# datatypevoid/babble

Hardware: AMD Instinct MI355X
Metric: consensus-ordered events/sec at N=256 peers (1 GPU and 8-GPU batched sims) (higher is better)
Workload: dtype int32

## Files before the change

### babble_amd/_lib.py

```python
from __future__ import annotations

import ctypes as C
import os

import numpy as np

HERE = os.path.dirname(os.path.abspath(__file__))
LIB_PATH = os.path.join(HERE, os.environ.get("HGX_LIB", "libhgx.so"))

_L = None


class HgxError(RuntimeError):

    def __init__(self, code: int, msg: str):
        super().__init__(msg)
        self.code = code
        self.msg = msg


class hgx_error(C.Structure):
    _fields_ = [("code", C.c_int32), ("msg", C.c_char * 252)]


# ... 134 lines not shown
    _sig(L, "hgx_last_round", i32, [p, i32])
    _sig(L, "hgx_round_event_count", i32, [p, i32, i32])
    _sig(L, "hgx_round_witnesses", i32, [p, i32, i32, p, i32])
    _sig(L, "hgx_known", i32, [p, i32, p])
    _sig(L, "hgx_consensus_events_count", i64, [p, i32])
    _sig(L, "hgx_consensus_events", i32, [p, i32, i64, i64, p])
    _sig(L, "hgx_num_blocks", i64, [p, i32])
    _sig(L, "hgx_block_info", i32, [p, i32, i64, p, p, p, p, p, p])
    _sig(L, "hgx_get_block", i32, [p, i32, i32, p, E])
    _sig(L, "hgx_consensus_received", i32, [p, i32, i64, i64, p, p, p])
    _sig(L, "hgx_last_from", i32, [p, i32, p, p, E])
    _sig(L, "hgx_participant_events", i32, [p, i32, i64, p, i64, p, E])
    _sig(L, "hgx_participant_event", i32, [p, i32, i64, p, E])
    _sig(L, "hgx_get_root", i32, [p, i32, p, p, p, p, E])
    _sig(L, "hgx_get_event", i32, [p, i64, p, p, p, p, p, p, p, E])
    _sig(L, "hgx_wire_info", i32, [p, i64, i64, p, p, p])
    _sig(L, "hgx_read_wire_info", i32, [p, i32, i64, i32, i64, p, p, E])
    _sig(L, "hgx_diff_wire", i32, [p, i32, p, i64, p, i64, C.POINTER(C.c_int64), C.POINTER(C.c_int32), E])
    _sig(L, "hgx_keep_bodies", i32, [p, i64, i64, E])
    _sig(L, "hgx_bodies_state", i32, [p, C.POINTER(C.c_int64), C.POINTER(C.c_int64), C.POINTER(C.c_int64)])
    _sig(L, "hgx_get_event_bodies", i32, [p, p, i64, p, p, p, i64, p, i64, C.POINTER(C.c_int64),
                                          C.POINTER(C.c_int64), E])
    _sig(L, "hgx_block_transactions", i32, [p, i32, i64, p, i64, p, i64, C.POINTER(C.c_int64),
                                            C.POINTER(C.c_int64), E])
    _sig(L, "hgx_get_block_hash", i32, [p, i32, i64, p, E])
    _sig(L, "hgx_block_hash_batch", i32, [i32, p, p, p, p, p, i64, p, E])
    _sig(L, "hgx_diff_wire_bodies", i32, [p, i32, p, i64, p, C.POINTER(hgx_wire_body_out), i64, C.POINTER(C.c_int64),
                                          C.POINTER(C.c_int64), C.POINTER(C.c_int64), C.POINTER(C.c_int32), E])
    _sig(L, "hgx_get_rounds", i32, [p, i64, i64, p, p, p])
    _sig(L, "hgx_get_received", i32, [p, i64, i64, p, p])
    _sig(L, "hgx_get_coords", i32, [p, i64, p, p])
    for nm in ("hgx_ancestor", "hgx_self_ancestor", "hgx_see", "hgx_strongly_see", "hgx_round", "hgx_witness"):
        _sig(L, nm, i32, [p, i64, i64] if nm not in ("hgx_round", "hgx_witness") else [p, i64])
    _sig(L, "hgx_oldest_self_ancestor_to_see", i64, [p, i64, i64])
    _sig(L, "hgx_block_hash", i32, [i64, i32, p, p, i32, p])
    _sig(L, "hgx_sha256_batch", i32, [i32, p, p, i64, p, p])
    _sig(L, "hgx_sha256_batch_device", i32, [p, p, i64, p, p])
    _sig(L, "hgx_p256_verify_batch", i32, [i32, p, i32, p, p, p, p, i64, p, p])
    _sig(L, "hgx_p256_verify_bench", i32, [i32, p, i32, p, p, p, p, i64, i32, i32, p, C.POINTER(C.c_double)])
    _sig(L, "hgx_sha256_bench", i32, [i32, i64, i32, i32, C.c_uint64, i32, i32, C.POINTER(C.c_double),
                                      C.POINTER(C.c_int64), C.POINTER(C.c_int64), i64, p])
    _sig(L, "hgx_phase_times", i32, [p, p, i32])
    _sig(L, "hgx_kernel_stats", i32, [p, i32, C.c_char_p, i32, C.POINTER(C.c_double), C.POINTER(C.c_int64),
                                      C.POINTER(C.c_double)])
    _sig(L, "hgx_reset_stats", i32, [p])
    _sig(L, "hgx_set_kernel_timing", i32, [p, i32])
    _sig(L, "hgx_set_coord_storage", i32, [p, i32])
    _sig(L, "hgx_set_fame_tally", i32, [p, i32])
    _sig(L, "hgx_set_round_kernel", i32, [p, i32])
    _sig(L, "hgx_set_sort_kernel", i32, [p, i32])
    _sig(L, "hgx_set_round_shards", i32, [p, i32])
    _sig(L, "hgx_set_shard_remote", i32, [p, i32])
    _sig(L, "hgx_exchange_floor_bench", i32, [i32, i32, i32, i32, C.POINTER(C.c_double)])
    _sig(L, "hgx_set_cts_kernel", i32, [p, i32])
    _sig(L, "hgx_set_root_others", i32, [p, p, i64, p])
    _sig(L, "hgx_set_la_kernel", i32, [p, i32])
    _sig(L, "hgx_set_ingest_pipeline", i32, [p, i32, i64])
    _sig(L, "hgx_set_incremental", i32, [p, i32])
    _sig(L, "hgx_find_order_begin", i32, [p, p])
    _sig(L, "hgx_find_order_end", i32, [p, p])
    _sig(L, "hgx_set_shard", i32, [p, i32, i32])
    _sig(L, "hgx_reset", i32, [p, p, p, p, p])
    _sig(L, "hgx_insert_wire_events", i32, [p, p, i64, p, p])
    _sig(L, "hgx_insert_wire_bodies", i32, [p, C.POINTER(hgx_wire_bodies), i64, p, p, p, C.POINTER(C.c_int64), E])
    _sig(L, "hgx_set_commit_callback", i32, [p, C.c_void_p, p])
    _sig(L, "hgx_get_frame", i32, [p, p, i64, p, p, p, p, p, p, p, i64, p, p])
    _sig(L, "hgx_prune_to_frame", i32, [p, p, i64, C.POINTER(C.c_int64), E])
    _sig(L, "hgx_get_root_ids", i32, [p, i32, p, C.POINTER(C.c_int32), p, C.POINTER(C.c_int32), E])
    _sig(L, "hgx_get_root_others", i32, [p, p, p, i64, C.POINTER(C.c_int64), E])
    _sig(L, "hgx_set_root_ids", i32, [p, p, p, p, p, p, p, i64, E])
    _sig(L, "hgx_shard_values", i64, [p, i32])
    _sig(L, "hgx_shard_export", i32, [p, p, i32])
    _sig(L, "hgx_shard_import", i32, [p, i32, p, i32])
    _sig(L, "hgx_reserve_rounds", i32, [p, i32])
    _sig(L, "hgx_device_alloc", i32, [i32, i64, C.POINTER(C.c_void_p)])
    _sig(L, "hgx_device_free", i32, [i32, p])
    _sig(L, "hgx_device_copy", i32, [i32, p, p, i64, i32])
    _L = L
    return L


def check(rc: int, err: hgx_error):
    if rc != 0:
        raise HgxError(int(err.code or rc), err.msg.decode(errors="replace"))
```

### babble_amd/csrc/hgx_device.h

```cpp
#pragma once

#include <hip/hip_runtime.h>

#include <cstdint>

namespace hgx {

__device__ __forceinline__ int lane_id() { return (int)(threadIdx.x & 63); }

__device__ __forceinline__ uint32_t block_excl_scan256(uint32_t v, uint32_t* sh, uint32_t* total) {
    const int lane = lane_id(), wave = threadIdx.x >> 6;
    uint32_t x = v;
    for (int o = 1; o < 64; o <<= 1) {
        const uint32_t y = __shfl_up(x, o);
        if (lane >= o) x += y;
    }
    if (lane == 63) sh[wave] = x;
    __syncthreads();
    uint32_t wbase = 0;
    for (int w = 0; w < wave; w++) wbase += sh[w];
    *total = sh[0] + sh[1] + sh[2] + sh[3];
    __syncthreads();
    return wbase + x - v;
}

template <int HD>
__device__ __forceinline__ uint32_t swar_ge_count(const uint32_t (&v)[HD], const uint32_t (&nf)[HD]) {
    uint32_t c = 0;
    if constexpr (HD % 2 == 0) {
#pragma unroll
        for (int i = 0; i < HD / 2; i++) {
            const uint64_t s = ((((uint64_t)v[2 * i + 1]) << 32) | v[2 * i]) + ((((uint64_t)nf[2 * i + 1]) << 32) | nf[2 * i]);
            c = __builtin_popcount((uint32_t)s & 0x80808080u) + c;
            asm volatile("" : "+v"(c));
            c = __builtin_popcount((uint32_t)(s >> 32) & 0x80808080u) + c;
            asm volatile("" : "+v"(c));
        }
    } else {
#pragma unroll
        for (int d = 0; d < HD; d++) c += __builtin_popcount((v[d] + nf[d]) & 0x80808080u);
    }
    return c;
}
__device__ __forceinline__ uint32_t swar_nf(uint32_t fd7) { return 0x80808080u - fd7; }

__device__ __forceinline__ uint64_t group_mask(int gs, int grp) {
    return (gs >= 64) ? ~0ull : (((1ull << gs) - 1ull) << (gs * grp));
}

template <typename CT>
struct Coord;
template <>
struct Coord<int32_t> {
    static constexpr int32_t kLaNone = -1;
    __device__ __forceinline__ static int32_t la(int32_t v) { return v; }
    __device__ __forceinline__ static int32_t enc_la(int32_t v) { return v; }
    __device__ __forceinline__ static int32_t fd(int32_t v) { return v; }
    __device__ __forceinline__ static int32_t enc_fd(int32_t v) { return v; }
};
template <>
struct Coord<uint16_t> {
    static constexpr int32_t kLaNone = 0;
    __device__ __forceinline__ static int32_t la(uint32_t v) { return (int32_t)v - 1; }
    __device__ __forceinline__ static uint16_t enc_la(int32_t v) { return (uint16_t)(v + 1); }
    __device__ __forceinline__ static int32_t fd(uint32_t v) { return v == 0xFFFFu ? 2147483647 : (int32_t)v; }
    __device__ __forceinline__ static uint16_t enc_fd(int32_t v) { return v >= 0xFFFF ? (uint16_t)0xFFFF : (uint16_t)v; }
};

__device__ __forceinline__ void wave_lds_fence() {
    __builtin_amdgcn_fence(__ATOMIC_SEQ_CST, "wavefront");
    __builtin_amdgcn_wave_barrier();
}

__device__ __forceinline__ uint64_t wave_min_u64(uint64_t x) {
    for (int o = 32; o >= 1; o >>= 1) {
        const uint64_t y = __shfl_xor(x, o);
        x = y < x ? y : x;
    }
    return x;
}

__device__ __forceinline__ uint64_t wave_max_u64(uint64_t x) {
    for (int o = 32; o >= 1; o >>= 1) {
        const uint64_t y = __shfl_xor(x, o);
        x = y > x ? y : x;
    }
    return x;
}

template <int CPL>
__device__ uint64_t wave_select_kth(const uint64_t (&v)[CPL], const bool (&ok)[CPL], int K,
                                    uint32_t* __restrict__ hist) {
    const int lane = lane_id();
    uint64_t lo = ~0ull, hi = 0;
#pragma unroll
    for (int q = 0; q < CPL; q++)
        if (ok[q]) { lo = v[q] < lo ? v[q] : lo; hi = v[q] > hi ? v[q] : hi; }
    lo = wave_min_u64(lo);
    hi = wave_max_u64(hi);
    bool act[CPL];
#pragma unroll
    for (int q = 0; q < CPL; q++) act[q] = ok[q];
    uint64_t base = lo;
    uint64_t range = hi - lo;
    int k = K;
    while (range != 0) {
        int bits = 64 - __clzll((long long)range);
        const int shift = bits > 8 ? bits - 8 : 0;
#pragma unroll
        for (int t = 0; t < 4; t++) hist[lane * 4 + t] = 0;
        wave_lds_fence();
#pragma unroll
        for (int q = 0; q < CPL; q++)
            if (act[q]) atomicAdd(&hist[(uint32_t)((v[q] - base) >> shift)], 1u);
        wave_lds_fence();
        uint32_t h[4], s = 0;
#pragma unroll
        for (int t = 0; t < 4; t++) { h[t] = hist[lane * 4 + t]; s += h[t]; }
        uint32_t incl = s;
        for (int o = 1; o < 64; o <<= 1) {
            const uint32_t y = __shfl_up(incl, o);
            if (lane >= o) incl += y;
        }
        const uint32_t excl = incl - s;
        int bucket = -1;
        uint32_t below = 0;
// ... 323 lines not shown
```

### babble_amd/csrc/hgx_kernels.hip

```cpp
#include <hip/hip_runtime.h>

#include <algorithm>
#include <cstdint>
#include <cstdlib>
#include <cstring>
#include <map>
#include <mutex>
#include <tuple>

#include "hgx_device.h"
#include "hgx_kernels.h"

namespace hgx {


constexpr int kLayoutB = 4096;
constexpr int kLayoutH = 1024;

__global__ void __launch_bounds__(256) k_ck_pack(int64_t E0, int64_t E, const int32_t* __restrict__ g_creator,
                                                 const int32_t* __restrict__ g_index, const int32_t* __restrict__ c_base,
                                                 int64_t* __restrict__ g_ck, const int32_t* __restrict__ gate) {
    if (gate && *gate) return;
    const int64_t gid = E0 + (int64_t)blockIdx.x * blockDim.x + threadIdx.x;
    if (gid >= E) return;
    const int c = g_creator[gid];
    g_ck[gid] = ((int64_t)c << 32) | (uint32_t)(g_index[gid] - c_base[c]);
}

__device__ __forceinline__ void layout_one(int64_t gid, int p, const int32_t* __restrict__ g_creator,
                                           const int64_t* __restrict__ g_ck, const int32_t* __restrict__ g_op,
                                           const int64_t* __restrict__ g_ts, const int32_t* __restrict__ g_rr,
                                           const int64_t* __restrict__ g_cts, const int32_t* __restrict__ c_off,
                                           const int32_t* __restrict__ c_base, int32_t* __restrict__ p_gid,
                                           int32_t* __restrict__ p_chain, int32_t* __restrict__ p_op,
                                           int32_t* __restrict__ p_opu, int32_t* __restrict__ p_opk,
                                           int64_t* __restrict__ p_ts, int32_t* __restrict__ p_rr,
                                           int64_t* __restrict__ p_cts, int C, int n, int seg) {
    const int c = g_creator[gid];
    const int op = g_op[gid];
    int opp = -1, opu = -1, opk = -1;
    if (op >= 0) {
        const int64_t ck = g_ck[op];
        const int oc = (int)(ck >> 32);
        const int ok = (int)(uint32_t)ck;
        opp = c_off[oc] + ok;
        opu = (ok / seg) * C + oc;
        opk = ((oc % n) << kOpkBits) | (ok & ((1 << kOpkBits) - 1));
    }
    p_opk[p] = opk;
    p_gid[p] = (int32_t)gid;
    p_chain[p] = c;
    p_op[p] = opp;
    p_opu[p] = opu;
    p_ts[p] = g_ts[gid];
    p_rr[p] = g_rr[gid];
    p_cts[p] = g_cts[gid];
}

__global__ void __launch_bounds__(256) k_layout_direct(int64_t E0, int64_t E, const int32_t* __restrict__ g_creator,
                                                       const int32_t* __restrict__ g_index, const int64_t* __restrict__ g_ck,
                                                       const int32_t* __restrict__ g_op,
                                                       const int64_t* __restrict__ g_ts, const int32_t* __restrict__ g_rr,
// ... 1366 lines not shown
                                                          uint32_t* __restrict__ segcur, uint64_t* __restrict__ kout,
                                                          uint32_t* __restrict__ vout) {
    const int i = blockIdx.x * blockDim.x + threadIdx.x;
    const bool v = i < m;
    int seg = -1, p = 0;
    uint64_t key = 0;
    if (v) {
        p = list[i];
        seg = (p_chain[p] / n) * R + p_rr[p];
        key = ((uint64_t)seg << cts_bits) | (uint64_t)(p_cts[p] - cmin);
    }
    bool head;
    int hl, len;
    wave_seg_runs(v, seg, head, hl, len);
    uint32_t base = 0;
    if (head) base = atomicAdd(&segcur[seg], (uint32_t)len);
    base = (uint32_t)__shfl((int)base, hl);
    if (v) {
        const uint32_t slot = segoff[seg] + base + (uint32_t)(lane_id() - hl);
        kout[slot] = key;
        vout[slot] = (uint32_t)p;
    }
}

__global__ void __launch_bounds__(256) k_seg_max(int nseg, const uint32_t* __restrict__ segc,
                                                 unsigned long long* __restrict__ out) {
    uint32_t mx = 0;
    for (int s = blockIdx.x * blockDim.x + threadIdx.x; s < nseg; s += gridDim.x * blockDim.x) mx = max(mx, segc[s]);
    for (int o = 32; o >= 1; o >>= 1) mx = max(mx, (uint32_t)__shfl_xor(mx, o));
    if (lane_id() == 0 && mx) atomicMax(out, (unsigned long long)mx);
}

__device__ __forceinline__ int cmp_s(const uint8_t* a, const uint8_t* b) {
    for (int k = 0; k < 32; k++)
        if (a[k] != b[k]) return a[k] < b[k] ? -1 : 1;
    return 0;
}

struct SortFinish {
    const int32_t* p_rr;
    const int64_t* p_cts;
    const int32_t* g_ntx;
    const uint8_t* g_loaded;
    const uint8_t* g_txnil;
    int32_t* order_gid;
    int32_t* g_rr;
    int64_t* g_cts;
    int32_t* blk_cnt;
    int64_t* blk_ntx;
    int32_t* blk_loaded;
    uint8_t* blk_nil;
};

template <int GS, int TB>
__global__ void __launch_bounds__(TB) k_seg_sort(int nseg, int seg0, int seg1, int32_t m, const uint32_t* __restrict__ segoff,
                                                  const uint64_t* __restrict__ kin, const uint32_t* __restrict__ vin,
                                                  const int32_t* __restrict__ p_gid, const uint8_t* __restrict__ g_S,
                                                  uint32_t* __restrict__ vout, int cap, SortFinish F) {
    extern __shared__ __attribute__((aligned(16))) uint64_t smem[];
    __shared__ int64_t red_ntx[TB / 64];
    __shared__ int32_t red_ld[TB / 64];
    constexpr int NG = TB / GS;
    const int grp = (int)threadIdx.x / GS, t = (int)threadIdx.x % GS;
    uint64_t* sk = smem + (size_t)grp * cap;
    uint32_t* sv = (uint32_t*)(smem + (size_t)NG * cap) + (size_t)grp * cap;
    uint16_t* rs = (uint16_t*)((uint32_t*)(smem + (size_t)NG * cap) + (size_t)NG * cap) + (size_t)grp * 2 * cap;
    auto sync = [&]() {
        if constexpr (GS == 64) wave_lds_fence(); else __syncthreads();
    };
    const int sgi = seg0 + (int)blockIdx.x * NG + grp;
    int o = 0, len = 0;
    if (sgi < seg1) {
        o = (int)segoff[sgi];
        len = (sgi + 1 < nseg ? (int)segoff[sgi + 1] : m) - o;
    }
    int64_t ntx = 0;
    int ld = 0;
    auto emit = [&](int i, uint32_t p) {
        vout[o + i] = p;
        const int gid = p_gid[p];
        F.order_gid[o + i] = gid;
        F.g_rr[gid] = F.p_rr[p];
        F.g_cts[gid] = F.p_cts[p];
        ntx += F.g_ntx[gid];
        ld += F.g_loaded[gid] ? 1 : 0;
        if (i == 0) F.blk_nil[sgi] = F.g_txnil[gid];
    };
    auto block_totals = [&]() {
        for (int w = 32; w >= 1; w >>= 1) {
            ntx += __shfl_xor(ntx, w);
            ld += __shfl_xor(ld, w);
        }
        if constexpr (GS > 64) {
            if (lane_id() == 0) { red_ntx[threadIdx.x >> 6] = ntx; red_ld[threadIdx.x >> 6] = ld; }
            __syncthreads();
            if (threadIdx.x == 0)
                for (int w = 1; w < TB / 64; w++) { ntx += red_ntx[w]; ld += red_ld[w]; }
        }
        if (t == 0 && len > 0) {
            F.blk_cnt[sgi] = len;
            F.blk_ntx[sgi] = ntx;
            F.blk_loaded[sgi] = ld;
        }
    };
    if (len <= 1) {
        if (len == 1 && t == 0) emit(0, vin[o]);
        block_totals();
        return;
    }
    int P = 2;
    while (P < len) P <<= 1;
    for (int i = t; i < P; i += GS) {
        sk[i] = i < len ? kin[o + i] : ~0ull;
        sv[i] = i < len ? vin[o + i] : 0u;
    }
    sync();
    for (int k = 2; k <= P; k <<= 1) {
        for (int j = k >> 1; j > 0; j >>= 1) {
            for (int q = t; q < (P >> 1); q += GS) {
                const int lo = 2 * j * (q / j) + (q & (j - 1)), hi = lo + j;
                const bool asc = (lo & k) == 0;
                const uint64_t a = sk[lo], b = sk[hi];
                if ((a > b) == asc) {
                    sk[lo] = b;
                    sk[hi] = a;
                    const uint32_t x = sv[lo];
                    sv[lo] = sv[hi];
                    sv[hi] = x;
                }
            }
            sync();
        }
    }
    bool tie_any = false;
    for (int i = t; i < len; i += GS) {
        const bool head = i == 0 || sk[i - 1] != sk[i];
        rs[i] = (uint16_t)(head ? i : 0);
        tie_any |= !head;
    }
    if constexpr (GS == 64) tie_any = __any(tie_any); else tie_any = __syncthreads_or(tie_any);
    if (!tie_any) {
        for (int i = t; i < len; i += GS) emit(i, sv[i]);
        block_totals();
        return;
    }
    sync();
    int cur = 0;
    for (int d = 1; d < len; d <<= 1) {
        const uint16_t* src = rs + cur * cap;
        uint16_t* dst = rs + (cur ^ 1) * cap;
        for (int i = t; i < len; i += GS) dst[i] = i >= d ? max(src[i], src[i - d]) : src[i];
        sync();
        cur ^= 1;
    }
    const uint16_t* st = rs + cur * cap;
    for (int i = t; i < len; i += GS) {
        const int s0 = st[i];
        const bool member = s0 != i || (i + 1 < len && st[i + 1] == i);
        if (member) {
            sk[i] = __builtin_bswap64(*(const uint64_t*)(g_S + (size_t)p_gid[sv[i]] * 32));
        }
    }
    sync();
    for (int i = t; i < len; i += GS) {
        const int s0 = st[i];
        const bool member = s0 != i || (i + 1 < len && st[i + 1] == i);
        if (!member) {
            emit(i, sv[i]);
            continue;
        }
        const uint64_t my = sk[i];
        const uint32_t vi = sv[i];
        const uint8_t* si = g_S + (size_t)p_gid[vi] * 32;
        int rank = 0;
        for (int jx = s0; jx < len && st[jx] == s0; jx++) {
            const uint64_t pj = sk[jx];
            const int c = pj != my ? (pj < my ? -1 : 1) : (jx == i ? 0 : cmp_s(g_S + (size_t)p_gid[sv[jx]] * 32, si));
            rank += c < 0 || (c == 0 && jx < i);
        }
        emit(s0 + rank, vi);
    }
    block_totals();
}

__global__ void __launch_bounds__(256) k_minmax_cts(int32_t m, const int32_t* __restrict__ list,
                                                    const int64_t* __restrict__ p_cts,
// ... 631 lines not shown
    const int nb = (m + kSortTile - 1) / kSortTile;
    hipLaunchKernelGGL(k_radix_hist, dim3(nb), dim3(kSortThreads), 0, s, kin, m, shift, a.hist, nb);
    scan_u32(s, a, a.hist, (int64_t)256 * nb);
    hipLaunchKernelGGL(k_radix_scatter, dim3(nb), dim3(kSortThreads), 0, s, kin, vin, m, shift, a.hist, nb, kout,
                       vout);
}

void launch_sort(hipStream_t s, const DevArrays& a, int32_t m, int64_t cmin, int cts_bits, int R, int n,
                 int seg_bits, uint32_t** final_vals, uint64_t** final_keys) {
    uint64_t *ka = a.key_a, *kb = a.key_b;
    uint32_t *va = a.val_a, *vb = a.val_b;
    if (cts_bits + seg_bits <= 64) {
        hipLaunchKernelGGL(k_keys_comb, dim3(nblk(m, 256)), dim3(256), 0, s, m, a.recv_list, a.p_cts, a.p_chain,
                           a.p_rr, cmin, cts_bits, R, n, ka, va);
        for (int sh = 0; sh < cts_bits + seg_bits; sh += 8) {
            radix_pass(s, a, m, sh, ka, va, kb, vb);
            uint64_t* tk = ka; ka = kb; kb = tk;
            uint32_t* tv = va; va = vb; vb = tv;
        }
        hipLaunchKernelGGL(k_tie_prefix, dim3(nblk(m, 256)), dim3(256), 0, s, m, va, ka, a.p_gid, a.g_S, kb);
        hipLaunchKernelGGL(k_tiefix_rank, dim3(nblk(m, 256)), dim3(256), 0, s, m, va, vb, ka, kb, a.p_gid, a.g_S);
        va = vb;
        *final_vals = va;
        *final_keys = ka;
        return;
    }
    hipLaunchKernelGGL(k_keys_cts, dim3(nblk(m, 256)), dim3(256), 0, s, m, a.recv_list, a.p_cts, cmin, ka, va);
    for (int sh = 0; sh < cts_bits; sh += 8) {
        radix_pass(s, a, m, sh, ka, va, kb, vb);
        uint64_t* tk = ka; ka = kb; kb = tk;
        uint32_t* tv = va; va = vb; vb = tv;
    }
    hipLaunchKernelGGL(k_keys_seg, dim3(nblk(m, 256)), dim3(256), 0, s, m, va, a.p_chain, a.p_rr, R, n, ka);
    for (int sh = 0; sh < seg_bits; sh += 8) {
        radix_pass(s, a, m, sh, ka, va, kb, vb);
        uint64_t* tk = ka; ka = kb; kb = tk;
        uint32_t* tv = va; va = vb; vb = tv;
    }
    hipLaunchKernelGGL(k_tiefix, dim3(nblk(m, 256)), dim3(256), 0, s, m, va, ka, a.p_cts, a.p_gid, a.g_S);
    *final_vals = va;
    *final_keys = ka;
}

int seg_sort_cap() { return kSegSortCap; }

void launch_seg_count(hipStream_t s, const DevArrays& a, int32_t m, int R, int n, int nseg, uint32_t* segc,
                      unsigned long long* max_out) {
    hipLaunchKernelGGL(k_seg_count_mm, dim3(std::min(2048u, nblk(m, 256))), dim3(256), 0, s, m, a.recv_list, a.p_cts,
                       a.p_chain, a.p_rr, R, n, segc, (unsigned long long*)a.minmax);
    hipLaunchKernelGGL(k_seg_max, dim3(std::max(1, std::min(256, (nseg + 255) / 256))), dim3(256), 0, s, nseg, segc,
                       max_out);
}

hipError_t launch_sort_seg(hipStream_t s, const DevArrays& a, int32_t m, int64_t cmin, int cts_bits, int R, int n,
                           int nseg, uint32_t* segoff, uint32_t* segcur, int max_seg, uint32_t** final_vals,
                           uint64_t** final_keys, const std::vector<int>* cuts,
                           const std::function<hipError_t(int)>& after_part) {
    uint64_t* kb = a.key_b;
    uint32_t *va = a.val_a, *vb = a.val_b;
    int cap = 2;
    while (cap < max_seg) cap <<= 1;
    if (cap > 512) {
        const hipError_t e = ensure_lds_limit((const void*)k_seg_sort<1024, 1024>, (size_t)cap * 16);
        if (e != hipSuccess) return e;
    }
    scan_u32(s, a, segoff, nseg);
    (void)hipMemsetAsync(segcur, 0, (size_t)nseg * 4, s);
    hipLaunchKernelGGL(k_seg_keys_scatter, dim3(nblk(m, 256)), dim3(256), 0, s, m, a.recv_list, a.p_cts, a.p_chain,
                       a.p_rr, cmin, cts_bits, R, n, segoff, segcur, kb, vb);
    const SortFinish F{a.p_rr, a.p_cts, a.g_ntx, a.g_loaded, a.g_txnil, a.order_gid, a.g_rr, a.g_cts,
                       a.blk_cnt, a.blk_ntx, a.blk_loaded, a.blk_nil};
    const int np = cuts ? (int)cuts->size() - 1 : 1;
    for (int k = 0; k < np; k++) {
        const int s0 = cuts ? (*cuts)[k] : 0, s1 = cuts ? (*cuts)[k + 1] : nseg;
        if (s1 > s0) {
            if (cap <= 512) {
                const size_t lds = (size_t)4 * cap * 16;
                hipLaunchKernelGGL((k_seg_sort<64, 256>), dim3((s1 - s0 + 3) / 4), dim3(256), lds, s, nseg, s0, s1, m,
                                   segoff, kb, vb, a.p_gid, a.g_S, va, cap, F);
            } else {
                const size_t lds = (size_t)cap * 16;
                hipLaunchKernelGGL((k_seg_sort<1024, 1024>), dim3(s1 - s0), dim3(1024), lds, s, nseg, s0, s1, m, segoff,
                                   kb, vb, a.p_gid, a.g_S, va, cap, F);
            }
        }
        if (after_part) {
            const hipError_t e = after_part(k);
            if (e != hipSuccess) return e;
        }
    }
    *final_vals = va;
    *final_keys = kb;
    return hipGetLastError();
}

void launch_root_floor(hipStream_t s, const DevArrays& a, const int32_t* root_round, int32_t* gfl, int32_t* gB,
                       int gmax, int C, int n, int max_len) {
    const int64_t work = (int64_t)C * max_len;
    if (work <= 0 || gmax < 0) return;
    if (a.compact)
        hipLaunchKernelGGL(k_root_floor<uint16_t>, dim3(nblk(work, 256)), dim3(256), 0, s, a.c_off, a.c_len, a.c_base,
                           root_round, (const uint16_t*)a.LA, gfl, C, n, max_len);
    else
        hipLaunchKernelGGL(k_root_floor<int32_t>, dim3(nblk(work, 256)), dim3(256), 0, s, a.c_off, a.c_len, a.c_base,
                           root_round, (const int32_t*)a.LA, gfl, C, n, max_len);
    hipLaunchKernelGGL(k_root_bound_init, dim3(nblk((int64_t)(gmax + 1) * C, 256)), dim3(256), 0, s, gB, a.c_len, C,
                       gmax);
    hipLaunchKernelGGL(k_root_bound, dim3(nblk(work, 256)), dim3(256), 0, s, a.c_off, a.c_len, gfl, gB, C, gmax,
                       max_len);
}

__global__ void k_round_first_gid(int r0, int R, int C, const int32_t* __restrict__ Bm, const uint8_t* __restrict__ wstat,
                                  const int32_t* __restrict__ c_off, const int32_t* __restrict__ p_gid,
                                  int32_t* __restrict__ first) {
    const int64_t t = (int64_t)blockIdx.x * blockDim.x + threadIdx.x;
    if (t >= (int64_t)(R - r0) * C) return;
    const int r = r0 + (int)(t / C), c = (int)(t % C);
    if (wstat[(size_t)r * C + c] != 2) return;
    atomicMin(&first[r - r0], p_gid[c_off[c] + Bm[(size_t)r * C + c]]);
}

void launch_round_first_gid(hipStream_t s, const DevArrays& a, int r0, int R, int C, int32_t* first) {
    if (R <= r0) return;
    hipLaunchKernelGGL(k_round_first_gid, dim3(nblk((int64_t)(R - r0) * C, 256)), dim3(256), 0, s, r0, R, C, a.Bm,
                       a.wstat, a.c_off, a.p_gid, first);
}

bool sort_small_ok(int32_t m) { return m <= kSortSmallMax; }

void launch_sort_small(hipStream_t s, const DevArrays& a, int32_t m, int n, uint32_t** final_vals) {
    const unsigned t = (unsigned)((m + kRankTile - 1) / kRankTile), tj = (unsigned)((m + kRankJT - 1) / kRankJT);
    hipLaunchKernelGGL(k_sort_rank, dim3(t, tj), dim3(kRankTile), 0, s, m, a.recv_list, a.p_cts, a.p_chain, a.p_rr,
                       a.p_gid, a.g_S, n, a.val_b);
    hipLaunchKernelGGL(k_sort_place, dim3(nblk(m, 256)), dim3(256), 0, s, m, a.recv_list, a.val_b, a.val_a);
    *final_vals = a.val_a;
}

void launch_finish_order(hipStream_t s, const DevArrays& a, int32_t m, const uint32_t* vals, int R, int n) {
    hipLaunchKernelGGL(k_finish_order, dim3(nblk(m, 256)), dim3(256), 0, s, m, vals, a.p_gid, a.p_chain, a.p_rr,
                       a.p_cts, a.g_ntx, a.g_loaded, a.g_txnil, R, n, a.order_gid, a.g_rr, a.g_cts, a.blk_cnt,
                       a.blk_ntx, a.blk_loaded, a.blk_nil);
}

void launch_gather_i32(hipStream_t s, int64_t E, const int32_t* src, const int32_t* g_pos, int32_t* dst) {
    if (E <= 0) return;
    hipLaunchKernelGGL(k_gather_i32, dim3(nblk(E, 256)), dim3(256), 0, s, E, src, g_pos, dst);
}
// ... 3 lines not shown
```

### babble_amd/hashgraph.py

```python
from __future__ import annotations

import ctypes as C
import os
from typing import List, Optional, Sequence

import numpy as np

from . import _lib
from ._lib import HgxError, hgx_error, hgx_events, ptr

UNKNOWN_PARENT = -2


def compact_columns(t) -> dict:
    ntx = np.where(np.asarray(t.txnil) != 0, -1, np.asarray(t.ntx)).astype(np.int32)
    return dict(creator=np.ascontiguousarray(t.creator, np.int32), index=np.ascontiguousarray(t.index, np.int32),
                sp=np.ascontiguousarray(t.sp, np.int32), op=np.ascontiguousarray(t.op, np.int32),
                ts=np.ascontiguousarray(t.ts, np.int64),
                coin=np.ascontiguousarray(np.asarray(t.hash)[:, 16] != 0, np.uint8),
                s=np.ascontiguousarray(t.s, np.uint8), ntx=ntx)


class HostBuffer:

# ... 967 lines not shown

def sha256_batch(data: np.ndarray, offsets: np.ndarray, device: int = 0) -> np.ndarray:
    data = np.ascontiguousarray(data, dtype=np.uint8)
    offsets = np.ascontiguousarray(offsets, dtype=np.int64)
    count = max(len(offsets) - 1, 0)
    out = np.zeros((count, 32), dtype=np.uint8)
    err = hgx_error()
    rc = _lib.lib().hgx_sha256_batch(device, ptr(data) if data.size else None, ptr(offsets) if count else None,
                                     count, ptr(out) if count else None, C.byref(err))
    _lib.check(rc, err)
    return out


def event_ids(bodies: Sequence[bytes], device: int = 0) -> List[bytes]:
    lens = np.fromiter((len(b) for b in bodies), dtype=np.int64, count=len(bodies))
    offsets = np.zeros(len(bodies) + 1, dtype=np.int64)
    np.cumsum(lens, out=offsets[1:])
    data = np.frombuffer(b"".join(bodies), dtype=np.uint8)
    return [bytes(r) for r in sha256_batch(data, offsets, device)]


def _splitmix64(x: np.ndarray) -> np.ndarray:
    with np.errstate(over="ignore"):
        z = x + np.uint64(0x9E3779B97F4A7C15)
        z = (z ^ (z >> np.uint64(30))) * np.uint64(0xBF58476D1CE4E5B9)
        z = (z ^ (z >> np.uint64(27))) * np.uint64(0x94D049BB133111EB)
        return z ^ (z >> np.uint64(31))


def sha256_bench_messages(n: int, min_len: int, max_len: int, seed: int) -> List[bytes]:
    i = np.arange(n, dtype=np.uint64)
    lens = min_len + (_splitmix64(~np.uint64(seed) + i) % np.uint64(max_len - min_len + 1)).astype(np.int64)
    total = int(lens.sum())
    words = _splitmix64(np.uint64(seed) + np.arange((total + 7) // 8, dtype=np.uint64))
    blob = words.astype("<u8").tobytes()
    out, o = [], 0
    for ln in lens:
        out.append(blob[o:o + int(ln)])
        o += int(ln)
    return out


def sha256_bench(count: int, min_len: int, max_len: int, seed: int = 5, warmup: int = 1, iters: int = 3,
                 n_sample: int = 64, device: int = 0) -> dict:
    ms, tot, nb = C.c_double(), C.c_int64(), C.c_int64()
    sample = np.zeros((n_sample, 32), dtype=np.uint8)
    rc = _lib.lib().hgx_sha256_bench(device, count, min_len, max_len, seed, warmup, iters, C.byref(ms),
                                     C.byref(tot), C.byref(nb), n_sample, ptr(sample))
    if rc:
        raise HgxError(rc, "hgx_sha256_bench failed")
    return {"ms_per_launch": ms.value, "bytes": tot.value, "blocks": nb.value, "sample": sample}


def _p256_cols(keys65, key_idx, digest, r, s):
    k = np.ascontiguousarray(keys65, np.uint8).reshape(-1, 65)
    cols = [np.ascontiguousarray(key_idx, np.int32)] + [np.ascontiguousarray(x, np.uint8).reshape(-1, 32)
                                                         for x in (digest, r, s)]
    m = cols[0].shape[0]
    assert all(c.shape[0] == m for c in cols[1:])
    return k, cols, m


def p256_verify(keys65, key_idx, digest, r, s, device: int = 0) -> np.ndarray:
    k, cols, m = _p256_cols(keys65, key_idx, digest, r, s)
    out = np.zeros(m, np.uint8)
    err = hgx_error()
    rc = _lib.lib().hgx_p256_verify_batch(device, ptr(k), k.shape[0], *[ptr(c) for c in cols], m, ptr(out),
                                          C.byref(err))
    _lib.check(rc, err)
    return out


def p256_verify_bench(keys65, key_idx, digest, r, s, warmup: int = 1, iters: int = 3, device: int = 0) -> dict:
    k, cols, m = _p256_cols(keys65, key_idx, digest, r, s)
    out = np.zeros(m, np.uint8)
    ms = C.c_double()
    rc = _lib.lib().hgx_p256_verify_bench(device, ptr(k), k.shape[0], *[ptr(c) for c in cols], m, warmup, iters,
                                          ptr(out), C.byref(ms))
    if rc:
        raise HgxError(rc, "hgx_p256_verify_bench failed")
    return {"ms_per_launch": ms.value, "out": out}
```

### include/hgx.h

```cpp
#ifndef HGX_H
#define HGX_H

#include <stdint.h>

#ifdef __cplusplus
extern "C" {
#endif

#define HGX_ABI_VERSION 6

enum {
    HGX_OK = 0,
    HGX_ERR_KEY_NOT_FOUND = 1,
    HGX_ERR_TOO_LATE = 2,
    HGX_ERR_PASSED_INDEX = 3,
    HGX_ERR_SKIPPED_INDEX = 4,
    HGX_ERR_NO_ROOT = 5,
    HGX_ERR_SELF_PARENT = 100,
    HGX_ERR_OTHER_PARENT = 101,
    HGX_ERR_INVALID = 102,
    HGX_ERR_CAPACITY = 103,
    HGX_ERR_SIGNATURE = 104,
    HGX_ERR_DEVICE = 200,
    HGX_ERR_PANIC = 300
// ... 218 lines not shown
} hgx_wire_out;
int32_t hgx_diff_wire(hgx_ctx* ctx, int32_t graph, const int32_t* known, int64_t sync_limit,
                      hgx_wire_out* out, int64_t cap, int64_t* count, int32_t* over_limit, hgx_error* err);

int32_t hgx_keep_bodies(hgx_ctx* ctx, int64_t tx_hint, int64_t bytes_hint, hgx_error* err);
int32_t hgx_bodies_state(hgx_ctx* ctx, int64_t* n_events, int64_t* n_tx, int64_t* n_bytes);
int32_t hgx_get_event_bodies(hgx_ctx* ctx, const int64_t* gids, int64_t count, uint8_t* sig_r, int32_t* ntx,
                             int64_t* tx_off, int64_t tx_cap, uint8_t* tx_bytes, int64_t bytes_cap, int64_t* n_tx,
                             int64_t* n_bytes, hgx_error* err);
int32_t hgx_block_transactions(hgx_ctx* ctx, int32_t graph, int64_t b, int64_t* tx_off, int64_t tx_cap,
                               uint8_t* tx_bytes, int64_t bytes_cap, int64_t* n_tx, int64_t* n_bytes, hgx_error* err);
int32_t hgx_get_block_hash(hgx_ctx* ctx, int32_t graph, int64_t b, uint8_t* out32, hgx_error* err);
int32_t hgx_block_hash_batch(int32_t device, const int64_t* round_received, const int32_t* ntx,
                             const int32_t* tx_nil, const int64_t* tx_off, const uint8_t* tx_bytes, int64_t count,
                             uint8_t* out32, hgx_error* err);
typedef struct {
    uint8_t* sig_r;
    int64_t* tx_off;
    int64_t tx_cap;
    uint8_t* tx_bytes;
    int64_t bytes_cap;
} hgx_wire_body_out;
int32_t hgx_diff_wire_bodies(hgx_ctx* ctx, int32_t graph, const int32_t* known, int64_t sync_limit,
                             hgx_wire_out* out, hgx_wire_body_out* body, int64_t cap, int64_t* count, int64_t* n_tx,
                             int64_t* n_bytes, int32_t* over_limit, hgx_error* err);

int32_t hgx_get_rounds(hgx_ctx* ctx, int64_t first, int64_t count, int32_t* round, int8_t* witness,
                       int8_t* famous);
int32_t hgx_get_received(hgx_ctx* ctx, int64_t first, int64_t count, int32_t* round_received,
                         int64_t* consensus_ts);
int32_t hgx_get_coords(hgx_ctx* ctx, int64_t gid, int32_t* last_ancestors, int32_t* first_descendants);

int32_t hgx_ancestor(hgx_ctx* ctx, int64_t x, int64_t y);
int32_t hgx_self_ancestor(hgx_ctx* ctx, int64_t x, int64_t y);
int32_t hgx_see(hgx_ctx* ctx, int64_t x, int64_t y);
int32_t hgx_strongly_see(hgx_ctx* ctx, int64_t x, int64_t y);
int64_t hgx_oldest_self_ancestor_to_see(hgx_ctx* ctx, int64_t x, int64_t y);
int32_t hgx_round(hgx_ctx* ctx, int64_t x);
int32_t hgx_witness(hgx_ctx* ctx, int64_t x);

int32_t hgx_block_hash(int64_t round_received, int32_t ntx, const uint8_t* const* tx, const int64_t* tx_len,
                       int32_t tx_nil, uint8_t* out32);

int32_t hgx_sha256_batch(int32_t device, const uint8_t* data, const int64_t* offsets, int64_t count,
                         uint8_t* out32, hgx_error* err);
int32_t hgx_sha256_batch_device(const uint8_t* d_data, const int64_t* d_offsets, int64_t count,
                                uint8_t* d_out32, void* stream);
int32_t hgx_sha256_bench(int32_t device, int64_t count, int32_t min_len, int32_t max_len, uint64_t seed,
                         int32_t warmup, int32_t iters, double* ms_per_launch, int64_t* total_bytes,
                         int64_t* n_blocks, int64_t n_sample, uint8_t* sample32);

int32_t hgx_exchange_floor_bench(int32_t device, int32_t chains, int32_t n, int32_t rounds, double* us_per_round);

int32_t hgx_p256_verify_batch(int32_t device, const uint8_t* keys65, int32_t n_keys, const int32_t* key_idx,
                              const uint8_t* digest32, const uint8_t* r32, const uint8_t* s32, int64_t count,
                              uint8_t* out, hgx_error* err);
int32_t hgx_p256_verify_bench(int32_t device, const uint8_t* keys65, int32_t n_keys, const int32_t* key_idx,
                              const uint8_t* digest32, const uint8_t* r32, const uint8_t* s32, int64_t count,
                              int32_t warmup, int32_t iters, uint8_t* out, double* ms_per_launch);

int32_t hgx_phase_times(hgx_ctx* ctx, double* out, int32_t cap);
int32_t hgx_kernel_stats(hgx_ctx* ctx, int32_t k, char* name, int32_t name_cap, double* ms, int64_t* launches,
                         double* bytes);
int32_t hgx_reset_stats(hgx_ctx* ctx);
int32_t hgx_set_kernel_timing(hgx_ctx* ctx, int32_t mask);

int32_t hgx_set_coord_storage(hgx_ctx* ctx, int32_t mode);
int32_t hgx_set_fame_tally(hgx_ctx* ctx, int32_t mode);
int32_t hgx_set_ingest_pipeline(hgx_ctx* ctx, int32_t pieces, int64_t min_events);
int32_t hgx_set_la_kernel(hgx_ctx* ctx, int32_t mode);
int32_t hgx_set_round_kernel(hgx_ctx* ctx, int32_t mode);
int32_t hgx_set_sort_kernel(hgx_ctx* ctx, int32_t mode);
int32_t hgx_set_round_shards(hgx_ctx* ctx, int32_t shards);
int32_t hgx_set_shard_remote(hgx_ctx* ctx, int32_t on);
int32_t hgx_set_cts_kernel(hgx_ctx* ctx, int32_t mode);
int32_t hgx_set_incremental(hgx_ctx* ctx, int32_t on);
int32_t hgx_reserve_rounds(hgx_ctx* ctx, int32_t rounds);

int32_t hgx_device_alloc(int32_t device, int64_t bytes, void** ptr);
int32_t hgx_device_free(int32_t device, void* ptr);
int32_t hgx_device_copy(int32_t device, void* dst, const void* src, int64_t bytes, int32_t to_device);

int32_t hgx_trace_gossip(int32_t n_participants, int32_t n_silent, int64_t n_events, uint64_t seed,
                         double stale_prob, int32_t stale_depth,
                         int32_t* creator, int64_t* index, int64_t* self_parent, int64_t* other_parent,
                         int64_t* timestamp_ns, uint8_t* hash, uint8_t* sig_s, int32_t* ntx, int32_t* tx_nil,
                         int64_t* tx_seq);
int32_t hgx_trace_tx_payload(int32_t creator, int64_t seq, uint8_t* out, int32_t cap);

#ifdef __cplusplus
}
#endif
#endif
```

Measured before the change: 284.8 million.

## Register-resident bitonic segment sort with DPP lane exchanges and packed key-index words

Rewrites the per-segment bitonic sort so each thread holds EPT elements in registers. Intra-thread stages use compare-swaps, intra-wave stages use DPP/swizzle lane exchanges, and only cross-wave stages go through LDS with barriers. When key bits plus log2(cap) fit in 64 bits, the value index is packed into the key's low bits, so only one word moves per compare and values are gathered once at the end. This removes most LDS traffic and barriers from the old shared-memory network, at the cost of a template explosion over EPT and PACK, higher register pressure, and a new host-callable correctness check entry point.

```diff
diff --git a/babble_amd/_lib.py b/babble_amd/_lib.py
--- a/babble_amd/_lib.py
+++ b/babble_amd/_lib.py
@@ -210,6 +210,7 @@
     _sig(L, "hgx_set_round_shards", i32, [p, i32])
     _sig(L, "hgx_set_shard_remote", i32, [p, i32])
     _sig(L, "hgx_exchange_floor_bench", i32, [i32, i32, i32, i32, C.POINTER(C.c_double)])
+    _sig(L, "hgx_seg_sort_check", i32, [i32, i32, p, i32, p, p, p, i32, p, C.POINTER(C.c_int32)])
     _sig(L, "hgx_set_cts_kernel", i32, [p, i32])
     _sig(L, "hgx_set_root_others", i32, [p, p, i64, p])
     _sig(L, "hgx_set_la_kernel", i32, [p, i32])
diff --git a/babble_amd/csrc/hgx_device.h b/babble_amd/csrc/hgx_device.h
--- a/babble_amd/csrc/hgx_device.h
+++ b/babble_amd/csrc/hgx_device.h
@@ -3,6 +3,8 @@
 #include <hip/hip_runtime.h>
 
 #include <cstdint>
+#include <type_traits>
+#include <utility>
 
 namespace hgx {
 
@@ -72,6 +74,29 @@
     __builtin_amdgcn_wave_barrier();
 }
 
+template <int... I, class F>
+__device__ __forceinline__ void static_for_seq(std::integer_sequence<int, I...>, F&& f) {
+    (f(std::integral_constant<int, I>{}), ...);
+}
+template <int N, class F>
+__device__ __forceinline__ void static_for(F&& f) {
+    static_for_seq(std::make_integer_sequence<int, N>{}, f);
+}
+
+template <int D>
+__device__ __forceinline__ uint32_t lane_xor_u32(uint32_t v) {
+    static_assert(D == 1 || D == 2 || D == 4 || D == 8 || D == 16 || D == 32, "lane distance");
+    if constexpr (D == 1) return (uint32_t)__builtin_amdgcn_update_dpp(0, (int)v, 0xB1, 0xF, 0xF, true);
+    else if constexpr (D == 2) return (uint32_t)__builtin_amdgcn_update_dpp(0, (int)v, 0x4E, 0xF, 0xF, true);
+    else if constexpr (D == 8) return (uint32_t)__builtin_amdgcn_update_dpp(0, (int)v, 0x128, 0xF, 0xF, true);
+    else if constexpr (D == 32) return (uint32_t)__shfl_xor((int)v, 32);
+    else return (uint32_t)__builtin_amdgcn_ds_swizzle((int)v, 0x1F | (D << 10));
+}
+template <int D>
+__device__ __forceinline__ uint64_t lane_xor_u64(uint64_t v) {
+    return ((uint64_t)lane_xor_u32<D>((uint32_t)(v >> 32)) << 32) | lane_xor_u32<D>((uint32_t)v);
+}
+
 __device__ __forceinline__ uint64_t wave_min_u64(uint64_t x) {
     for (int o = 32; o >= 1; o >>= 1) {
         const uint64_t y = __shfl_xor(x, o);
diff --git a/babble_amd/csrc/hgx_kernels.hip b/babble_amd/csrc/hgx_kernels.hip
--- a/babble_amd/csrc/hgx_kernels.hip
+++ b/babble_amd/csrc/hgx_kernels.hip
@@ -8,6 +8,7 @@
 #include <mutex>
 #include <tuple>
 
+#include "hgx.h"
 #include "hgx_device.h"
 #include "hgx_kernels.h"
 
@@ -1480,7 +1481,14 @@
     uint8_t* blk_nil;
 };
 
-template <int GS, int TB>
+template <bool PACK>
+__device__ __forceinline__ void seg_cx(uint64_t& a, uint32_t& va, uint64_t b, uint32_t vb, bool keep_min) {
+    const bool take = PACK ? (b < a) == keep_min : (keep_min ? b < a : b > a);
+    a = take ? b : a;
+    if constexpr (!PACK) va = take ? vb : va;
+}
+
+template <int GS, int TB, int EPT, bool PACK>
 __global__ void __launch_bounds__(TB) k_seg_sort(int nseg, int seg0, int seg1, int32_t m, const uint32_t* __restrict__ segoff,
                                                   const uint64_t* __restrict__ kin, const uint32_t* __restrict__ vin,
                                                   const int32_t* __restrict__ p_gid, const uint8_t* __restrict__ g_S,
@@ -1489,6 +1497,8 @@
     __shared__ int64_t red_ntx[TB / 64];
     __shared__ int32_t red_ld[TB / 64];
     constexpr int NG = TB / GS;
+    constexpr int CAP = GS * EPT;
+    constexpr int LOGCAP = __builtin_ctz(CAP);
     const int grp = (int)threadIdx.x / GS, t = (int)threadIdx.x % GS;
     uint64_t* sk = smem + (size_t)grp * cap;
     uint32_t* sv = (uint32_t*)(smem + (size_t)NG * cap) + (size_t)grp * cap;
@@ -1538,28 +1548,103 @@
     }
     int P = 2;
     while (P < len) P <<= 1;
-    for (int i = t; i < P; i += GS) {
-        sk[i] = i < len ? kin[o + i] : ~0ull;
-        sv[i] = i < len ? vin[o + i] : 0u;
-    }
+    const int ib = EPT * t;
+    uint64_t w[EPT];
+    uint32_t v[EPT];
+    static_for<EPT>([&](auto E) {
+        constexpr int e = decltype(E)::value;
+        const int i = ib + e;
+        w[e] = ~0ull;
+        v[e] = 0u;
+        if (i < len) {
+            const uint64_t key = kin[o + i];
+            if constexpr (PACK) {
+                w[e] = (key << LOGCAP) | (uint64_t)i;
+            } else {
+                w[e] = key;
+                v[e] = vin[o + i];
+            }
+        }
+    });
+    [[maybe_unused]] int flip = 0;
+    static_for<LOGCAP>([&](auto LK) {
+        constexpr int k = 2 << decltype(LK)::value;
+        if (k <= P) {
+            static_for<decltype(LK)::value + 1>([&](auto JJ) {
+                constexpr int j = (k >> 1) >> decltype(JJ)::value;
+                if constexpr (j < EPT) {
+                    static_for<EPT>([&](auto E) {
+                        constexpr int e = decltype(E)::value;
+                        if constexpr ((e & j) == 0) {
+                            bool asc;
+                            if constexpr (k < EPT) asc = (e & k) == 0; else asc = (ib & k) == 0;
+                            const bool sw = PACK ? (w[e] > w[e + j]) == asc : (asc ? w[e] > w[e + j] : w[e] < w[e + j]);
+                            const uint64_t a = w[e], b = w[e + j];
+                            w[e] = sw ? b : a;
+                            w[e + j] = sw ? a : b;
+                            if constexpr (!PACK) {
+                                const uint32_t x = v[e], y = v[e + j];
+                                v[e] = sw ? y : x;
+                                v[e + j] = sw ? x : y;
+                            }
+                        }
+                    });
+                } else if constexpr (j < 64 * EPT) {
+                    const bool keep_min = ((ib & j) == 0) == ((ib & k) == 0);
+                    static_for<EPT>([&](auto E) {
+                        constexpr int e = decltype(E)::value;
+                        const uint64_t b = lane_xor_u64<j / EPT>(w[e]);
+                        uint32_t vb = 0u;
+                        if constexpr (!PACK) vb = lane_xor_u32<j / EPT>(v[e]);
+                        seg_cx<PACK>(w[e], v[e], b, vb, keep_min);
+                    });
+                } else {
+                    const bool keep_min = ((ib & j) == 0) == ((ib & k) == 0);
+                    const bool in = ib < P;
+                    if constexpr (PACK) {
+                        uint64_t* xb = smem + (flip ? CAP : 0);
+                        flip ^= 1;
+                        if (in) static_for<EPT>([&](auto E) { xb[ib + decltype(E)::value] = w[decltype(E)::value]; });
+                        __syncthreads();
+                        if (in)
+                            static_for<EPT>([&](auto E) {
+                                constexpr int e = decltype(E)::value;
+                                seg_cx<PACK>(w[e], v[e], xb[(ib ^ j) + e], 0u, keep_min);
+                            });
+                    } else {
+                        if (in)
+                            static_for<EPT>([&](auto E) {
+                                constexpr int e = decltype(E)::value;
+                                sk[ib + e] = w[e];
+                                sv[ib + e] = v[e];
+                            });
+                        __syncthreads();
+                        if (in)
+                            static_for<EPT>([&](auto E) {
+                                constexpr int e = decltype(E)::value;
+                                seg_cx<PACK>(w[e], v[e], sk[(ib ^ j) + e], sv[(ib ^ j) + e], keep_min);
+                            });
+                        __syncthreads();
+                    }
+                }
+            });
+        }
+    });
+    if constexpr (PACK && GS > 64) __syncthreads();
+    static_for<EPT>([&](auto E) {
+        constexpr int e = decltype(E)::value;
+        const int i = ib + e;
+        if (i < len) {
+            if constexpr (PACK) {
+                sk[i] = w[e] >> LOGCAP;
+                sv[i] = vin[o + (int)(w[e] & (uint64_t)(CAP - 1))];
+            } else {
+                sk[i] = w[e];
+                sv[i] = v[e];
+            }
+        }
+    });
     sync();
-    for (int k = 2; k <= P; k <<= 1) {
-        for (int j = k >> 1; j > 0; j >>= 1) {
-            for (int q = t; q < (P >> 1); q += GS) {
-                const int lo = 2 * j * (q / j) + (q & (j - 1)), hi = lo + j;
-                const bool asc = (lo & k) == 0;
-                const uint64_t a = sk[lo], b = sk[hi];
-                if ((a > b) == asc) {
-                    sk[lo] = b;
-                    sk[hi] = a;
-                    const uint32_t x = sv[lo];
-                    sv[lo] = sv[hi];
-                    sv[hi] = x;
-                }
-            }
-            sync();
-        }
-    }
     bool tie_any = false;
     for (int i = t; i < len; i += GS) {
         const bool head = i == 0 || sk[i - 1] != sk[i];
@@ -2297,6 +2382,54 @@
                        max_out);
 }
 
+namespace {
+struct SegSortArgs {
+    int nseg, s0, s1;
+    int32_t m;
+    const uint32_t* segoff;
+    const uint64_t* kin;
+    const uint32_t* vin;
+    const int32_t* p_gid;
+    const uint8_t* g_S;
+    uint32_t* vout;
+    int cap;
+    SortFinish F;
+};
+
+template <int GS, int TB, int EPT, bool PACK>
+hipError_t seg_sort_go(hipStream_t s, const SegSortArgs& g, bool launch) {
+    constexpr int NG = TB / GS;
+    const size_t lds = (size_t)NG * g.cap * 16;
+    if (!launch) return GS > 64 ? ensure_lds_limit((const void*)k_seg_sort<GS, TB, EPT, PACK>, lds) : hipSuccess;
+    hipLaunchKernelGGL((k_seg_sort<GS, TB, EPT, PACK>), dim3((g.s1 - g.s0 + NG - 1) / NG), dim3(TB), lds, s, g.nseg, g.s0,
+                       g.s1, g.m, g.segoff, g.kin, g.vin, g.p_gid, g.g_S, g.vout, g.cap, g.F);
+    return hipSuccess;
+}
+
+template <int GS, int TB, bool PACK>
+hipError_t seg_sort_ept(hipStream_t s, const SegSortArgs& g, bool launch) {
+    switch (std::max(1, g.cap / GS)) {
+        case 1: return seg_sort_go<GS, TB, 1, PACK>(s, g, launch);
+        case 2: return seg_sort_go<GS, TB, 2, PACK>(s, g, launch);
+        case 4: return seg_sort_go<GS, TB, 4, PACK>(s, g, launch);
+        case 8: return seg_sort_go<GS, TB, 8, PACK>(s, g, launch);
+        default: return hipErrorInvalidValue;
+    }
+}
+
+bool seg_sort_packs(int cap, int key_bits) {
+    int lc = 6;
+    while ((1 << lc) < cap) lc++;
+    return key_bits + lc <= 64;
+}
+
+hipError_t seg_sort_run(hipStream_t s, const SegSortArgs& g, bool pack, bool launch) {
+    if (g.cap <= 512)
+        return pack ? seg_sort_ept<64, 256, true>(s, g, launch) : seg_sort_ept<64, 256, false>(s, g, launch);
+    return pack ? seg_sort_ept<1024, 1024, true>(s, g, launch) : seg_sort_ept<1024, 1024, false>(s, g, launch);
+}
+}
+
 hipError_t launch_sort_seg(hipStream_t s, const DevArrays& a, int32_t m, int64_t cmin, int cts_bits, int R, int n,
                            int nseg, uint32_t* segoff, uint32_t* segcur, int max_seg, uint32_t** final_vals,
                            uint64_t** final_keys, const std::vector<int>* cuts,
@@ -2305,30 +2438,24 @@
     uint32_t *va = a.val_a, *vb = a.val_b;
     int cap = 2;
     while (cap < max_seg) cap <<= 1;
-    if (cap > 512) {
-        const hipError_t e = ensure_lds_limit((const void*)k_seg_sort<1024, 1024>, (size_t)cap * 16);
+    if (cap > kSegSortCap) return hipErrorInvalidValue;
+    SegSortArgs g{nseg, 0, nseg, m, segoff, kb, vb, a.p_gid, a.g_S, va, cap,
+                  SortFinish{a.p_rr, a.p_cts, a.g_ntx, a.g_loaded, a.g_txnil, a.order_gid, a.g_rr, a.g_cts,
+                             a.blk_cnt, a.blk_ntx, a.blk_loaded, a.blk_nil}};
+    const bool pack = seg_sort_packs(cap, cts_bits);
+    {
+        const hipError_t e = seg_sort_run(s, g, pack, false);
         if (e != hipSuccess) return e;
     }
     scan_u32(s, a, segoff, nseg);
     (void)hipMemsetAsync(segcur, 0, (size_t)nseg * 4, s);
     hipLaunchKernelGGL(k_seg_keys_scatter, dim3(nblk(m, 256)), dim3(256), 0, s, m, a.recv_list, a.p_cts, a.p_chain,
                        a.p_rr, cmin, cts_bits, R, n, segoff, segcur, kb, vb);
-    const SortFinish F{a.p_rr, a.p_cts, a.g_ntx, a.g_loaded, a.g_txnil, a.order_gid, a.g_rr, a.g_cts,
-                       a.blk_cnt, a.blk_ntx, a.blk_loaded, a.blk_nil};
     const int np = cuts ? (int)cuts->size() - 1 : 1;
     for (int k = 0; k < np; k++) {
-        const int s0 = cuts ? (*cuts)[k] : 0, s1 = cuts ? (*cuts)[k + 1] : nseg;
-        if (s1 > s0) {
-            if (cap <= 512) {
-                const size_t lds = (size_t)4 * cap * 16;
-                hipLaunchKernelGGL((k_seg_sort<64, 256>), dim3((s1 - s0 + 3) / 4), dim3(256), lds, s, nseg, s0, s1, m,
-                                   segoff, kb, vb, a.p_gid, a.g_S, va, cap, F);
-            } else {
-                const size_t lds = (size_t)cap * 16;
-                hipLaunchKernelGGL((k_seg_sort<1024, 1024>), dim3(s1 - s0), dim3(1024), lds, s, nseg, s0, s1, m, segoff,
-                                   kb, vb, a.p_gid, a.g_S, va, cap, F);
-            }
-        }
+        g.s0 = cuts ? (*cuts)[k] : 0;
+        g.s1 = cuts ? (*cuts)[k + 1] : nseg;
+        if (g.s1 > g.s0) (void)seg_sort_run(s, g, pack, true);
         if (after_part) {
             const hipError_t e = after_part(k);
             if (e != hipSuccess) return e;
@@ -2338,6 +2465,83 @@
     *final_keys = kb;
     return hipGetLastError();
 }
+
+hipError_t seg_sort_check_run(hipStream_t s, int nseg, int32_t m, int max_seg, int key_bits, bool force_kv,
+                              const uint32_t* segoff, const uint64_t* kin, const uint32_t* vin, const int32_t* p_gid,
+                              const uint8_t* g_S, uint32_t* vout, const SortFinish& F, bool* packed) {
+    int cap = 2;
+    while (cap < max_seg) cap <<= 1;
+    if (cap > kSegSortCap) return hipErrorInvalidValue;
+    const SegSortArgs g{nseg, 0, nseg, m, segoff, kin, vin, p_gid, g_S, vout, cap, F};
+    *packed = !force_kv && seg_sort_packs(cap, key_bits);
+    hipError_t e = seg_sort_run(s, g, *packed, false);
+    if (e == hipSuccess) e = seg_sort_run(s, g, *packed, true);
+    return e == hipSuccess ? hipGetLastError() : e;
+}
+
+}
+
+extern "C" int32_t hgx_seg_sort_check(int32_t device, int32_t nseg, const uint32_t* segoff, int32_t m,
+                                      const uint64_t* keys, const uint32_t* vals, const uint8_t* S32,
+                                      int32_t force_kv, uint32_t* out_vals, int32_t* packed_out) {
+    if (nseg < 1 || m < 1 || !segoff || !keys || !vals || !S32 || !out_vals) return HGX_ERR_INVALID;
+    int64_t max_seg = 0;
+    uint64_t all = 0;
+    if (segoff[0] != 0) return HGX_ERR_INVALID;
+    for (int sg = 0; sg < nseg; sg++) {
+        const int64_t b = segoff[sg], e = sg + 1 < nseg ? (int64_t)segoff[sg + 1] : (int64_t)m;
+        if (e < b || e > m) return HGX_ERR_INVALID;
+        max_seg = std::max(max_seg, e - b);
+    }
+    for (int32_t i = 0; i < m; i++) {
+        if (vals[i] >= (uint32_t)m) return HGX_ERR_INVALID;
+        all |= keys[i];
+    }
+    if (max_seg > hgx::seg_sort_cap()) return HGX_ERR_INVALID;
+    int key_bits = 0;
+    while (key_bits < 64 && (all >> key_bits) != 0) key_bits++;
+    int prev = 0;
+    (void)hipGetDevice(&prev);
+    if (hipSetDevice(device) != hipSuccess) return HGX_ERR_DEVICE;
+    const size_t M = (size_t)m, NS = (size_t)nseg;
+    const size_t o_keys = 0, o_cts = o_keys + 8 * M, o_gcts = o_cts + 8 * M, o_bntx = o_gcts + 8 * M,
+                 o_S = o_bntx + 8 * NS, o_vin = o_S + 32 * M, o_vout = o_vin + 4 * M, o_gid = o_vout + 4 * M,
+                 o_prr = o_gid + 4 * M, o_ntx = o_prr + 4 * M, o_ogid = o_ntx + 4 * M, o_grr = o_ogid + 4 * M,
+                 o_off = o_grr + 4 * M, o_bcnt = o_off + 4 * NS, o_bld = o_bcnt + 4 * NS, o_ld = o_bld + 4 * NS,
+                 o_nil = o_ld + M, o_bnil = o_nil + M, total = o_bnil + NS;
+    uint8_t* d = nullptr;
+    hipStream_t s = nullptr;
+    bool packed = false;
+    std::vector<int32_t> ident(M);
+    for (int32_t i = 0; i < m; i++) ident[(size_t)i] = i;
+    hipError_t e = hipStreamCreateWithFlags(&s, hipStreamNonBlocking);
+    if (e == hipSuccess) e = hipMalloc((void**)&d, total);
+    if (e == hipSuccess) e = hipMemsetAsync(d, 0, total, s);
+    if (e == hipSuccess) e = hipMemcpyAsync(d + o_keys, keys, 8 * M, hipMemcpyHostToDevice, s);
+    if (e == hipSuccess) e = hipMemcpyAsync(d + o_S, S32, 32 * M, hipMemcpyHostToDevice, s);
+    if (e == hipSuccess) e = hipMemcpyAsync(d + o_vin, vals, 4 * M, hipMemcpyHostToDevice, s);
+    if (e == hipSuccess) e = hipMemcpyAsync(d + o_gid, ident.data(), 4 * M, hipMemcpyHostToDevice, s);
+    if (e == hipSuccess) e = hipMemcpyAsync(d + o_off, segoff, 4 * NS, hipMemcpyHostToDevice, s);
+    if (e == hipSuccess) {
+        const hgx::SortFinish F{(const int32_t*)(d + o_prr), (const int64_t*)(d + o_cts), (const int32_t*)(d + o_ntx),
+                                d + o_ld, d + o_nil, (int32_t*)(d + o_ogid), (int32_t*)(d + o_grr),
+                                (int64_t*)(d + o_gcts), (int32_t*)(d + o_bcnt), (int64_t*)(d + o_bntx),
+                                (int32_t*)(d + o_bld), d + o_bnil};
+        e = hgx::seg_sort_check_run(s, nseg, m, (int)max_seg, key_bits, force_kv != 0, (const uint32_t*)(d + o_off),
+                                    (const uint64_t*)(d + o_keys), (const uint32_t*)(d + o_vin),
+                                    (const int32_t*)(d + o_gid), d + o_S, (uint32_t*)(d + o_vout), F, &packed);
+    }
+    if (e == hipSuccess) e = hipMemcpyAsync(out_vals, d + o_vout, 4 * M, hipMemcpyDeviceToHost, s);
+    if (e == hipSuccess) e = hipStreamSynchronize(s);
+    if (d) (void)hipFree(d);
+    if (s) (void)hipStreamDestroy(s);
+    (void)hipSetDevice(prev);
+    if (e != hipSuccess) return HGX_ERR_DEVICE;
+    if (packed_out) *packed_out = packed ? 1 : 0;
+    return HGX_OK;
+}
+
+namespace hgx {
 
 void launch_root_floor(hipStream_t s, const DevArrays& a, const int32_t* root_round, int32_t* gfl, int32_t* gB,
                        int gmax, int C, int n, int max_len) {
diff --git a/babble_amd/hashgraph.py b/babble_amd/hashgraph.py
--- a/babble_amd/hashgraph.py
+++ b/babble_amd/hashgraph.py
@@ -1043,6 +1043,22 @@
     return {"ms_per_launch": ms.value, "bytes": tot.value, "blocks": nb.value, "sample": sample}
 
 
+def seg_sort_check(segoff, keys, vals, S, force_kv: bool = False, device: int = 0):
+    so = np.ascontiguousarray(segoff, np.uint32)
+    k = np.ascontiguousarray(keys, np.uint64)
+    v = np.ascontiguousarray(vals, np.uint32)
+    s = np.ascontiguousarray(S, np.uint8).reshape(-1, 32)
+    m = k.shape[0]
+    assert v.shape[0] == m and s.shape[0] == m
+    out = np.zeros(m, np.uint32)
+    packed = C.c_int32()
+    rc = _lib.lib().hgx_seg_sort_check(device, so.shape[0], ptr(so), m, ptr(k), ptr(v), ptr(s), int(bool(force_kv)),
+                                       ptr(out), C.byref(packed))
+    if rc:
+        raise HgxError(rc, "hgx_seg_sort_check failed")
+    return out, bool(packed.value)
+
+
 def _p256_cols(keys65, key_idx, digest, r, s):
     k = np.ascontiguousarray(keys65, np.uint8).reshape(-1, 65)
     cols = [np.ascontiguousarray(key_idx, np.int32)] + [np.ascontiguousarray(x, np.uint8).reshape(-1, 32)
diff --git a/include/hgx.h b/include/hgx.h
--- a/include/hgx.h
+++ b/include/hgx.h
@@ -294,6 +294,10 @@
 
 int32_t hgx_exchange_floor_bench(int32_t device, int32_t chains, int32_t n, int32_t rounds, double* us_per_round);
 
+int32_t hgx_seg_sort_check(int32_t device, int32_t nseg, const uint32_t* segoff, int32_t m, const uint64_t* keys,
+                           const uint32_t* vals, const uint8_t* S32, int32_t force_kv, uint32_t* out_vals,
+                           int32_t* packed_out);
+
 int32_t hgx_p256_verify_batch(int32_t device, const uint8_t* keys65, int32_t n_keys, const int32_t* key_idx,
                               const uint8_t* digest32, const uint8_t* r32, const uint8_t* s32, int64_t count,
                               uint8_t* out, hgx_error* err);
```

After: 288.5 million (median of 6 runs). 1.3% higher.
